# MartinBeseda/FEM-ElastoPlasticity

Measured on NVIDIA B200. Metric: K_tangent assembly Melem/s + DP return-map Mpts/s + PCG-Newton s/step; %HBM roof, higher is better.
Workload: dtype f64

## Files before the change

fem_elastoplasticity_b200/_lib.py:

```python
import ctypes as C
import os

_HERE = os.path.dirname(os.path.abspath(__file__))
LIB_PATH = os.environ.get("FEM_B200_LIB") or os.path.join(_HERE, "libfem_b200.so")

STATUS = {0: "FEM_OK", 1: "FEM_ERR_INVALID_ARG", 2: "FEM_ERR_CUDA", 3: "FEM_ERR_NONFINITE_JACOBIAN",
          4: "FEM_ERR_PCG_BREAKDOWN", 5: "FEM_ERR_PCG_MAXIT", 6: "FEM_ERR_UNSUPPORTED", 7: "FEM_ERR_NO_DEVICE"}
FEM_ERR_PCG_MAXIT = 5


class FemError(RuntimeError):
    def __init__(self, code, msg):
        super().__init__(f"{STATUS.get(code, code)}: {msg}")
        self.code = code


class NonFiniteJacobian(FemError, ArithmeticError):
    pass


_vp, _i64, _i32, _dbl = C.c_void_p, C.c_int64, C.c_int, C.c_double

SIGNATURES = {
    "fem_last_error_string": [],
# ... 27 lines not shown
    "fem_ppcg_begin": [_vp, _vp, _i32, _vp],
    "fem_ppcg_spmv_dot": [_vp, _vp, _vp, _vp, _vp, _vp, C.POINTER(_vp), _i32, _i32, _vp],
    "fem_ppcg_update_xr": [_vp, _vp, _vp, _vp, _vp, _vp, _vp, C.POINTER(_vp), _i32, _i32, _vp],
    "fem_ppcg_update_p": [_vp, _i64, _i64, _vp, _vp, _vp, _i64, _i64, _vp, _i64, _i64, _vp, _vp, C.POINTER(_vp), _i32, _i32, _vp],
    "fem_pcg": [_vp, _vp, _vp, _vp, _dbl, _i32, _i32, _vp, _vp, C.POINTER(_i32), C.POINTER(_dbl), _vp],
    "fem_coarse_galerkin": [_vp, _vp, _vp, _vp, _vp, _dbl, _dbl, _dbl, _dbl, _i32, _i32, _vp, _vp],
    "fem_dense_gemv": [_i32, _vp, _vp, _vp, _vp, _vp],
    "fem_tl_init": [_i64, _vp, _vp, _vp, _vp, _vp, _dbl, _dbl, _dbl, _dbl, _i32, _i32, _vp, _vp, _vp, _vp],
    "fem_tl_update_xr": [_i64, _vp, _vp, _vp, _vp, _dbl, _dbl, _dbl, _dbl, _i32, _i32, _vp, _vp, _vp, _vp, _i32, _vp],
    "fem_tl_apply": [_i64, _i32, _vp, _vp, _vp, _vp, _dbl, _dbl, _dbl, _dbl, _i32, _i32, _vp, _vp, _vp, _i32, _i32, _vp],
    "fem_mg_sizeof": [_i32],
    "fem_mg_lattice": [_i64, _vp, _dbl, _dbl, _dbl, _dbl, _i32, _i32, _i32, _vp, _vp, _vp, _vp],
    "fem_mg_galerkin_fine": [_vp, _vp, _vp, _vp, _vp, _i32, _vp, _i32, _i32, _i32, _i32, _i32, _vp, _vp, _vp],
    "fem_mg_galerkin_stencil": [_i32, _i32, _i32, _i32, _vp, _i32, _i32, _i32, _i32, _i32, _vp, _vp],
    "fem_mg_block_jacobi": [_vp, _vp, _vp, _vp, _vp],
    "fem_mg_level_finalize": [_i64, _vp, _dbl, _vp, _vp],
    "fem_mg_stencil_apply": [_i32, _i32, _i32, _i32, _vp, _vp, _vp, _vp],
    "fem_mg_stencil_to_dense": [_i32, _i32, _vp, _vp, _vp],
    "fem_mg_vcycle": [_vp, _vp, _vp, _vp, _vp, _vp, _vp],
    "fem_peer_allreduce": [_vp, _i32, _vp, C.POINTER(_vp), _i64, _i64, _i64, _i32, _i32, _vp],
    "fem_mg_fine_step": [_vp, _vp, _i32, _vp, _vp, _vp, _vp, _dbl, _dbl, _vp, _vp],
    "fem_mg_to_f32": [_i64, _vp, _vp, _vp],
    "fem_mg_exchange_run": [_vp, _vp, _vp, _vp],
    "fem_mg_pcg_init": [_i64, _vp, _vp, _vp, _vp, _vp, _vp],
    "fem_mg_pcg_update_xr": [_i64, _vp, _vp, _vp, _vp, _vp, _i32, _vp],
    "fem_mg_pcg_update_p": [_i64, _vp, _vp, _vp, _i32, _vp],
    "fem_energy_norms": [_vp, _vp, _vp, _vp, _vp, _vp, _vp, _vp],
    "fem_vec_axpby": [_i64, _dbl, _vp, _dbl, _vp, _vp, _vp],
    "fem_transform": [_vp, _vp, _vp, _vp],
    "fem_vector_volume": [_vp, _vp, C.POINTER(_dbl), _vp, _vp],
    "fem_segment_sum_ordered": [_i64, _vp, _vp, _vp, _vp],
    "fem_midpoints_p2_count": [_i64, _i64, _vp, C.POINTER(_vp), C.POINTER(_i64), C.POINTER(_i64), C.POINTER(_i32), _vp],
    "fem_midpoints_p2_fill": [_vp, _vp, _vp, _vp, _vp, _vp, _vp],
    "fem_midpoints_p2_destroy": [_vp, _vp],
    "fem_set_tuning": [C.c_char_p, _i32],
}
_RESTYPE = {"fem_last_error_string": C.c_char_p, "fem_plan_bytes": _i64}

_lib = None


def load():
    global _lib
    if _lib is not None:
        return _lib
    if not os.path.isfile(LIB_PATH):
        raise ImportError(f"{LIB_PATH} not found: build it with `python -c 'import __graft_entry__ as g; g.build()'` "
                          "(there is no CPU fallback)")
    lib = C.CDLL(LIB_PATH)
    for name, args in SIGNATURES.items():
# ... 6 lines not shown
        if lib.fem_set_tuning(k.strip().encode(), int(v)) != 0:
            raise ValueError(f"FEM_B200_TUNING: unknown key {k!r}")
    return lib


def check(code):
    if code != 0:
        msg = load().fem_last_error_string().decode()
        if code == 3:
            raise NonFiniteJacobian(code, msg)
        raise FemError(code, msg)


def call(name, *args):
    check(getattr(load(), name)(*args))
```

fem_elastoplasticity_b200/csrc/common.cuh:

```cuda
#pragma once
#include <cuda.h>
#include <cuda_runtime.h>
#include <stdint.h>
#include <stdio.h>
#include <string.h>

#include "../../include/fem_b200.h"

#define FEM_MAX_NP 8
#define FEM_MAX_NQ 9
#define FEM_WARP 32
#define FEM_INVALID_KEY 0xFFFFFFFFu
#define FEM_SLICE_COUNTERS 64
#define FEM_SPMV_TILE 256
#define FEM_SPMV_THREADS (2 * FEM_SPMV_TILE)
#define FEM_SPMV_MAXSEG 4
#define FEM_SPMV_CAP 1024
#define FEM_SPMV_DESC 12
#define FEM_STAGE_MAXBOXW 96
int fem_encode_rows_map(CUtensorMap* out, const double* base, int64_t n_int, int rows, int boxw);

void fem_set_error(const char* fmt, ...);

struct FemTuning {
  int return_map_variant;
  int assemble_warps;
  int spmv_group;
  int spmv_blocks_per_sm;
  int assemble_variant;
  int spmv_unroll;
  int spmv_staged;
  int peer_timeout_ms;
  int assemble_canon;
  int strain_variant;
  int mg_stencil_sym;
  int peer_nowait;
};
extern FemTuning g_fem_tuning;

#define FEM_CUDA_CHECK(expr)                                                                     \
  do {                                                                                           \
    cudaError_t _e = (expr);                                                                     \
    if (_e != cudaSuccess) {                                                                     \
      fem_set_error("%s failed at %s:%d: %s", #expr, __FILE__, __LINE__, cudaGetErrorString(_e)); \
      return FEM_ERR_CUDA;                                                                       \
    }                                                                                            \
  } while (0)

#define FEM_REQUIRE(cond, msg)                                    \
  do {                                                            \
// ... 126 lines not shown
```

fem_elastoplasticity_b200/csrc/mg.cu:

```cuda
#include "common.cuh"
#include "spmv.cuh"
#include "spmv_stream.cuh"
#include "peer.cuh"

struct fem_peer_table {
  void* p[FEM_MG_MAX_PEERS];
};

namespace {

struct Geom {
  int nxn, nrows, g0, nrows_global;
  int64_t n;
};
static Geom geom_of(const fem_mg_level& L) { return Geom{L.nxn, L.nrows, L.g0, L.nrows_global, (int64_t)L.nxn * L.nrows}; }

__device__ __forceinline__ double w1(int o) { return o ? 0.5 : 1.0; }

__global__ void mg_lattice_kernel(int64_t n_n, const double* __restrict__ coord, double x0, double y0, double ihx, double ihy, int LX,
                                  int lat_rows, int g0, int32_t* lat, int32_t* __restrict__ node_lat, int32_t* err) {
  for (int64_t a = (int64_t)blockIdx.x * blockDim.x + threadIdx.x; a < n_n; a += (int64_t)gridDim.x * blockDim.x) {
    const double fx = (coord[a] - x0) * ihx, fy = (coord[n_n + a] - y0) * ihy;
    const long long ix = llrint(fx), iy = llrint(fy) - g0;
    if (fabs(fx - (double)ix) > 1e-6 || fabs(fy - (double)(iy + g0)) > 1e-6 || ix < 0 || ix >= LX || iy < 0 || iy >= lat_rows) {
// ... 159 lines not shown
      if (nbr_idx[p0 + j] == a) {
        k00 = vals[4 * (int64_t)p0 + 2 * j];
        k01 = vals[4 * (int64_t)p0 + 2 * j + 1];
        k10 = vals[4 * (int64_t)p0 + 2 * deg + 2 * j];
        k11 = vals[4 * (int64_t)p0 + 2 * deg + 2 * j + 1];
        break;
      }
    const bool f0 = mask ? mask[2 * a] != 0 : true, f1 = mask ? mask[2 * a + 1] != 0 : true;
    double2 ia, ib;
    block_inverse(k00, 0.5 * (k01 + k10), k11, f0, f1, ia, ib);
    dinv[a] = ia;
    dinv[n_n + a] = ib;
  }
}

__global__ void mg_stencil_to_dense_kernel(Geom g, const double* __restrict__ S, double* __restrict__ A) {
  const int64_t t = (int64_t)blockIdx.x * blockDim.x + threadIdx.x;
  if (t >= g.n * 9) return;
  const int64_t node = t / 9;
  const int s = (int)(t % 9);
  const int i = (int)(node % g.nxn), j = (int)(node / g.nxn);
  const int ii = i + s % 3 - 1, jj = j + s / 3 - 1;
  if (ii < 0 || ii >= g.nxn || jj < 0 || jj >= g.nrows) return;
  const int64_t nb = ii + (int64_t)jj * g.nxn, nc = 2 * g.n;
#pragma unroll
  for (int q = 0; q < 4; ++q) A[(2 * node + (q >> 1)) * nc + 2 * nb + (q & 1)] = S[(int64_t)(4 * s + q) * g.n + node];
}

enum { MG_APPLY = 0, MG_RESID = 1, MG_CHEB = 2, MG_FIRST = 3 };

// ... 199 lines not shown
    ordered_accumulate<1>(v, dst, rb);
  }
}

__global__ void __launch_bounds__(256) mg_fine_first_kernel(int64_t lo, int64_t hi, int64_t n_n, const double2* __restrict__ b,
                                                            const double2* __restrict__ dinv, double2* __restrict__ d, double2* __restrict__ out,
                                                            double c2) {
  for (int64_t i = lo + (int64_t)blockIdx.x * blockDim.x + threadIdx.x; i < hi; i += (int64_t)gridDim.x * blockDim.x) {
    const double2 bi = b[i], da = dinv[i], db = dinv[n_n + i];
    const double2 dn = make_double2(c2 * (da.x * bi.x + da.y * bi.y), c2 * (db.x * bi.x + db.y * bi.y));
    d[i] = dn;
    out[i] = dn;
  }
}

template <bool LAT>
__global__ void __launch_bounds__(256) mg_restrict_kernel(Geom c, int row_lo, int row_hi, int nxf, int nrows_f, int g0f, int nrows_global_f,
                                                          const int32_t* __restrict__ lat, const double2* __restrict__ r, double2* __restrict__ bc) {
  const int64_t t = (int64_t)blockIdx.x * blockDim.x + threadIdx.x;
  if (t >= (int64_t)(row_hi - row_lo) * c.nxn) return;
  const int I = (int)(t % c.nxn), J = row_lo + (int)(t / c.nxn), Jg = J + c.g0;
  double a0 = 0.0, a1 = 0.0;
#pragma unroll
  for (int db = -1; db <= 1; ++db) {
    const int fjg = 2 * Jg + db, fj = fjg - g0f;
    if (fjg < 0 || fjg >= nrows_global_f || fj < 0 || fj >= nrows_f) continue;
#pragma unroll
    for (int da = -1; da <= 1; ++da) {
      const int fi = 2 * I + da;
      if (fi < 0 || fi >= nxf) continue;
// ... 37 lines not shown
  const int64_t node = (int64_t)row_lo * f.nxn + t;
  const int i = (int)(node % f.nxn), j = (int)(node / f.nxn);
  const double2 z = prolong_point(c, i, j + f.g0, xc);
  double2 v = xf[node];
  v.x += z.x;
  v.y += z.y;
  xf[node] = v;
}

__global__ void __launch_bounds__(256) mg_prolong_fine_kernel(int64_t n_n, const int32_t* __restrict__ node_lat, int LX, int g0,
                                                              const uint8_t* __restrict__ mask, Geom c, const double2* xc, double2* __restrict__ xf) {
  for (int64_t a = (int64_t)blockIdx.x * blockDim.x + threadIdx.x; a < n_n; a += (int64_t)gridDim.x * blockDim.x) {
    uchar2 mk = make_uchar2(1, 1);
    if (mask) mk = reinterpret_cast<const uchar2*>(mask)[a];
    if (!mk.x && !mk.y) continue;
    const int la = node_lat[a];
    const double2 z = prolong_point(c, la % LX, la / LX + g0, xc);
    double2 v = xf[a];
    if (mk.x) v.x += z.x;
    if (mk.y) v.y += z.y;
    xf[a] = v;
  }
}

__global__ void __launch_bounds__(256) mg_exchange_kernel(const fem_mg_exchange ex, const double2* __restrict__ v, uint64_t* err, uint64_t timeout_ns) {
  __shared__ int sh_last;
  int64_t total = 0;
  for (int k = 0; k < ex.n_send; ++k) total += ex.count[k];
  for (int64_t t = (int64_t)blockIdx.x * blockDim.x + threadIdx.x; t < total; t += (int64_t)gridDim.x * blockDim.x) {
    int64_t o = t;
    int k = 0;
// ... 184 lines not shown
    if (sh.group == 4) MGT(4);
    else if (sh.group == 8) MGT(8);
    else MGT(16);
#undef MGT
  } else {
#define MGR(G) mg_fine_rows_kernel<G, MODE, VT><<<sh.blocks, 256, 0, st>>>(P->n_n, P->nbr_ptr, P->nbr_idx, K, x, epi, dot, rb)
    if (sh.group == 4) MGR(4);
    else if (sh.group == 8) MGR(8);
    else MGR(16);
#undef MGR
  }
  FEM_CUDA_CHECK(cudaGetLastError());
  return FEM_OK;
}

template <int MODE>
int launch_fine(const fem_plan* P, const fem_mg_desc* D, const double* K, const double* b, const double* x, double* out, double c1, double c2,
                double* dot, cudaStream_t st) {
  if (D->K32) return launch_fine_vt<MODE, float>(P, D, D->K32, b, x, out, c1, c2, dot, st);
  return launch_fine_vt<MODE, double>(P, D, K, b, x, out, c1, c2, dot, st);
}

__global__ void __launch_bounds__(256) mg_to_f32_kernel(int64_t n4, const double4* __restrict__ src, float4* __restrict__ dst) {
  for (int64_t i = (int64_t)blockIdx.x * blockDim.x + threadIdx.x; i < n4; i += (int64_t)gridDim.x * blockDim.x) {
    const double2 a = __ldcs(reinterpret_cast<const double2*>(src + i)), b = __ldcs(reinterpret_cast<const double2*>(src + i) + 1);
    __stcs(dst + i, make_float4((float)a.x, (float)a.y, (float)b.x, (float)b.y));
  }
}

#define MG_TRY(expr)             \
  do {                           \
    const int _rc = (expr);      \
    if (_rc != FEM_OK) return _rc; \
// ... 88 lines not shown
  const int64_t items = (int64_t)(row_hi - row_lo) * nxc;
  if (items <= 0) return FEM_OK;
  mg_galerkin_stencil_kernel<<<grid_for(items, 128), 128, 0, (cudaStream_t)stream>>>(f, Sf, c, row_lo, row_hi, Sc);
  FEM_CUDA_CHECK(cudaGetLastError());
  return FEM_OK;
}

extern "C" int fem_mg_block_jacobi(const fem_plan* P, const double* K_vals, const uint8_t* mask, double* dinv, fem_stream stream) {
  FEM_REQUIRE(P && K_vals && dinv, "null pointer");
  mg_block_jacobi_kernel<<<grid_for(P->n_n), 256, 0, (cudaStream_t)stream>>>(P->n_n, P->nbr_ptr, P->nbr_idx, K_vals, mask,
                                                                             reinterpret_cast<double2*>(dinv));
  FEM_CUDA_CHECK(cudaGetLastError());
  return FEM_OK;
}

extern "C" int fem_mg_level_finalize(int64_t n, double* S, double thresh, double* dinv, fem_stream stream) {
  FEM_REQUIRE(S && dinv && n > 0, "null pointer");
  mg_level_finalize_kernel<<<grid_for(n), 256, 0, (cudaStream_t)stream>>>(n, S, thresh, reinterpret_cast<double2*>(dinv));
  FEM_CUDA_CHECK(cudaGetLastError());
  return FEM_OK;
}

extern "C" int fem_mg_stencil_apply(int nxn, int nrows, int row_lo, int row_hi, const double* S, const double* x, double* y, fem_stream stream) {
  FEM_REQUIRE(S && x && y && nxn > 0 && nrows > 0 && row_lo >= 0 && row_hi <= nrows, "null pointer or bad rows");
  const Geom g{nxn, nrows, 0, nrows, (int64_t)nxn * nrows};
  const int64_t items = (int64_t)(row_hi - row_lo) * nxn;
  if (items <= 0) return FEM_OK;
  mg_stencil_kernel<MG_APPLY, double, false><<<grid_for(items), 256, 0, (cudaStream_t)stream>>>(g, row_lo, row_hi, S, reinterpret_cast<const double2*>(x), nullptr,
                                                                                 nullptr, nullptr, reinterpret_cast<double2*>(y), 0.0, 0.0);
  FEM_CUDA_CHECK(cudaGetLastError());
// ... 33 lines not shown
  peer_allreduce_kernel<<<1, 256, 0, (cudaStream_t)stream>>>(vals, n, reinterpret_cast<uint64_t*>(comm), tab, lines_word, seq_word, err_word, rank, world,
                                                            timeout_ns);
  FEM_CUDA_CHECK(cudaGetLastError());
  return FEM_OK;
}

extern "C" int fem_mg_vcycle(const fem_plan* P, const fem_mg_desc* D, const double* K_vals, const double* r, double* z, double* dot,
                             fem_stream stream) {
  FEM_REQUIRE(P && D && K_vals && r && z, "null pointer");
  FEM_REQUIRE(D->n_levels >= 1 && D->n_levels <= FEM_MG_MAX_LEVELS && D->degree >= 1 && D->degree <= FEM_MG_MAX_DEGREE, "levels / degree");
  FEM_REQUIRE(D->lat && D->node_lat && D->dinv && D->xa && D->xb && D->d && D->r && D->coarse_inv, "descriptor");
  FEM_REQUIRE(D->own_node_lo >= 0 && D->own_node_hi <= P->n_n && D->own_node_lo < D->own_node_hi, "owned node range");
  cudaStream_t st = (cudaStream_t)stream;
  const int k = D->degree;
  const int64_t n2 = P->n_n;
  double *cur = D->xa, *oth = D->xb;
  const fem_mg_exchange *ecur = &D->ex_xa, *eoth = &D->ex_xb;
  auto swap = [&]() { double* t = cur; cur = oth; oth = t; const fem_mg_exchange* e = ecur; ecur = eoth; eoth = e; };
  mg_fine_first_kernel<<<vgrid(n2, P->sm_count), 256, 0, st>>>(D->own_node_lo, D->own_node_hi, n2, reinterpret_cast<const double2*>(r), reinterpret_cast<const double2*>(D->dinv),
                                                              reinterpret_cast<double2*>(D->d), reinterpret_cast<double2*>(cur), D->c2[0]);
  FEM_CUDA_CHECK(cudaGetLastError());
  for (int s = 1; s < k; ++s) {
    MG_TRY(run_exchange(*ecur, cur, D->err, st));
    MG_TRY(launch_fine<MG_CHEB>(P, D, K_vals, r, cur, oth, D->c1[s], D->c2[s], nullptr, st));
    swap();
  }
  MG_TRY(run_exchange(*ecur, cur, D->err, st));
  MG_TRY(launch_fine<MG_RESID>(P, D, K_vals, r, cur, D->r, 0.0, 0.0, nullptr, st));
  MG_TRY(run_exchange(D->ex_r, D->r, D->err, st));
  const fem_mg_level& C = D->lev[0];
  {
    const Geom c = geom_of(C);
    const int64_t items = (int64_t)(C.res_hi - C.res_lo) * C.nxn;
    if (items > 0) {
      mg_restrict_kernel<true><<<grid_for(items), 256, 0, st>>>(c, C.res_lo, C.res_hi, D->LX, D->lat_rows, D->g0, D->nrows_global, D->lat,
                                                                reinterpret_cast<const double2*>(D->r), reinterpret_cast<double2*>(C.b));
      FEM_CUDA_CHECK(cudaGetLastError());
    }
    MG_TRY(run_exchange(C.ex_b, C.b, D->err, st));
  }
  const double* xc = nullptr;
  MG_TRY(vcycle_level(D, 0, &xc, st));
  MG_TRY(run_exchange(xc == C.xa ? C.ex_xa : C.ex_xb, xc, D->err, st));
  mg_prolong_fine_kernel<<<vgrid(n2, P->sm_count), 256, 0, st>>>(n2, D->node_lat, D->LX, D->g0, D->mask, geom_of(C), reinterpret_cast<const double2*>(xc),
                                                                reinterpret_cast<double2*>(cur));
  FEM_CUDA_CHECK(cudaGetLastError());
  for (int s = 0; s < k; ++s) {
    const bool last = s == k - 1;
    MG_TRY(run_exchange(*ecur, cur, D->err, st));
    MG_TRY(launch_fine<MG_CHEB>(P, D, K_vals, r, cur, last ? z : oth, s == 0 ? 0.0 : D->c1[s], D->c2[s], last ? dot : nullptr, st));
    swap();
  }
  return FEM_OK;
}

extern "C" int fem_mg_fine_step(const fem_plan* P, const fem_mg_desc* D, int mode, const double* K_vals, const double* b, const double* x,
                                double* out, double c1, double c2, double* dot, fem_stream stream) {
  FEM_REQUIRE(P && D && K_vals && b && x && out && (mode == MG_RESID || mode == MG_CHEB) && out != x, "arguments");
  cudaStream_t st = (cudaStream_t)stream;
// ... 29 lines not shown
```

fem_elastoplasticity_b200/csrc/plan.cu:

```cuda
#include <stdarg.h>

#include <vector>

#include "common.cuh"

static thread_local char g_err[512] = "no error";
void fem_set_error(const char* fmt, ...) {
  va_list ap;
  va_start(ap, fmt);
  vsnprintf(g_err, sizeof(g_err), fmt, ap);
  va_end(ap);
}
extern "C" const char* fem_last_error_string(void) { return g_err; }
extern "C" int fem_version(void) { return 100; }

FemTuning g_fem_tuning = {};
extern "C" int fem_set_tuning(const char* key, int value) {
  FEM_REQUIRE(key != nullptr, "key");
  if (!strcmp(key, "return_map_variant")) g_fem_tuning.return_map_variant = value;
  else if (!strcmp(key, "assemble_warps")) g_fem_tuning.assemble_warps = value;
  else if (!strcmp(key, "spmv_group")) g_fem_tuning.spmv_group = value;
  else if (!strcmp(key, "spmv_blocks_per_sm")) g_fem_tuning.spmv_blocks_per_sm = value;
  else if (!strcmp(key, "assemble_variant")) g_fem_tuning.assemble_variant = value;
  else if (!strcmp(key, "spmv_unroll")) g_fem_tuning.spmv_unroll = value;
  else if (!strcmp(key, "spmv_staged")) g_fem_tuning.spmv_staged = value;
  else if (!strcmp(key, "peer_timeout_ms")) g_fem_tuning.peer_timeout_ms = value;
  else if (!strcmp(key, "peer_nowait")) g_fem_tuning.peer_nowait = value;
  else if (!strcmp(key, "strain_variant")) g_fem_tuning.strain_variant = value;
  else if (!strcmp(key, "assemble_canon")) g_fem_tuning.assemble_canon = value;
  else if (!strcmp(key, "mg_stencil_sym")) g_fem_tuning.mg_stencil_sym = value;
  else {
    fem_set_error("unknown tuning key %s", key);
    return FEM_ERR_INVALID_ARG;
  }
  return FEM_OK;
}

extern "C" int fem_device_info(int* sm_count, int* cc_major, int* cc_minor, int64_t* free_bytes, int64_t* total_bytes) {
  int dev = 0, n = 0;
  if (cudaGetDeviceCount(&n) != cudaSuccess || n == 0) {
    fem_set_error("no CUDA device visible");
    return FEM_ERR_NO_DEVICE;
  }
  FEM_CUDA_CHECK(cudaGetDevice(&dev));
  if (sm_count) FEM_CUDA_CHECK(cudaDeviceGetAttribute(sm_count, cudaDevAttrMultiProcessorCount, dev));
  if (cc_major) FEM_CUDA_CHECK(cudaDeviceGetAttribute(cc_major, cudaDevAttrComputeCapabilityMajor, dev));
  if (cc_minor) FEM_CUDA_CHECK(cudaDeviceGetAttribute(cc_minor, cudaDevAttrComputeCapabilityMinor, dev));
  size_t f = 0, t = 0;
  FEM_CUDA_CHECK(cudaMemGetInfo(&f, &t));
// ... 866 lines not shown
```

fem_elastoplasticity_b200/mg.py:

```python
import ctypes as C
import time

import torch

from ._lib import call, load
from .plan import _ptr, _stream

MAX_LEVELS, MAX_DEGREE, MAX_PEERS = 16, 8, 16


class MultigridUnsupported(ValueError):
    pass


class Exchange(C.Structure):
    _fields_ = [("n_send", C.c_int32), ("n_wait", C.c_int32), ("src_off", C.c_int64 * MAX_PEERS), ("count", C.c_int64 * MAX_PEERS),
                ("dst", C.c_void_p * MAX_PEERS), ("dst_flag", C.c_void_p * MAX_PEERS), ("wait_flag", C.c_void_p * MAX_PEERS),
                ("seq", C.c_void_p)]


class Level(C.Structure):
    _fields_ = [("nxn", C.c_int32), ("nrows", C.c_int32), ("g0", C.c_int32), ("own_lo", C.c_int32), ("own_hi", C.c_int32),
                ("nrows_global", C.c_int32), ("res_lo", C.c_int32), ("res_hi", C.c_int32),
                ("S", C.c_void_p), ("S32", C.c_void_p), ("dinv", C.c_void_p), ("b", C.c_void_p), ("xa", C.c_void_p), ("xb", C.c_void_p), ("d", C.c_void_p),
                ("r", C.c_void_p), ("c1", C.c_double * MAX_DEGREE), ("c2", C.c_double * MAX_DEGREE),
                ("ex_xa", Exchange), ("ex_xb", Exchange), ("ex_r", Exchange), ("ex_b", Exchange)]


class Desc(C.Structure):
    _fields_ = [("n_levels", C.c_int32), ("degree", C.c_int32), ("LX", C.c_int32), ("lat_rows", C.c_int32), ("g0", C.c_int32),
                ("nrows_global", C.c_int32), ("lat", C.c_void_p), ("node_lat", C.c_void_p), ("own_node_lo", C.c_int64),
                ("own_node_hi", C.c_int64), ("mask", C.c_void_p), ("dinv", C.c_void_p), ("xa", C.c_void_p), ("xb", C.c_void_p),
                ("d", C.c_void_p), ("r", C.c_void_p), ("c1", C.c_double * MAX_DEGREE), ("c2", C.c_double * MAX_DEGREE),
                ("ex_xa", Exchange), ("ex_xb", Exchange), ("ex_r", Exchange), ("lev", Level * MAX_LEVELS), ("coarse_inv", C.c_void_p),
                ("K32", C.c_void_p), ("err", C.c_void_p)]


def chebyshev_coefficients(lmax, ratio, degree):
    lmin = lmax / ratio
    theta, delta = 0.5 * (lmax + lmin), 0.5 * (lmax - lmin)
    sigma = theta / delta
    rho = 1.0 / sigma
    c1, c2 = [0.0], [1.0 / theta]
    for _ in range(1, degree):
        rho_new = 1.0 / (2.0 * sigma - rho)
        c1.append(rho_new * rho)
        c2.append(2.0 * rho_new / delta)
        rho = rho_new
    return c1, c2

# ... 102 lines not shown
            self._make_arena(n)
        a = self._vec
        self.r, self.q, self.x, self.z = (z(n) for _ in range(4))
        self.minv = z(2 * n)
        self.p = a("p", n)
        self.scal = z(8)
        self.v0 = {"xa": a("xa0", n), "xb": a("xb0", n), "d": z(n), "r": a("r0", n)}
        self.lv = []
        for li, lay in enumerate(self.layouts):
            g0l, nrows, own_lo, own_hi, res_lo, res_hi = lay["ranks"][rank]
            nn = lay["nxn"] * nrows
            self.lv.append({"nxn": lay["nxn"], "nrows": nrows, "g0": g0l, "own": (own_lo, own_hi), "res": (res_lo, res_hi), "n": nn,
                            "N": lay["nrows_global"], "rep": lay["replicated"], "first_rep": lay["first_replicated"],
                            "S": z(36 * nn), "dinv": z(4 * nn), "d": z(2 * nn), "b": a(f"b{li + 1}", 2 * nn),
                            "xa": a(f"xa{li + 1}", 2 * nn), "xb": a(f"xb{li + 1}", 2 * nn), "r": a(f"r{li + 1}", 2 * nn), "lmax": None})
        self.coarse_inv, self.desc, self.setup_seconds, self.lmax0 = None, None, None, None
        self._graph, self._graph_key = None, None
        self.launches_last = 0

    def _vec(self, name, size):
        if name in self._arena_slots:
            off, _ = self._arena_slots[name]
            return self.arena[off:off + size]
        return torch.zeros(size, dtype=torch.float64, device=self.device)

    def _make_arena(self, n):
        import torch.distributed as dist
        import torch.distributed._symmetric_memory as symm
        dev, world = self.device, self.world
        nmax = torch.tensor([n], dtype=torch.int64, device=dev)
# ... 132 lines not shown
        for li in range(1, self.n_levels):
            f, c = self.lv[li - 1], self.lv[li]
            rows = c["res"] if c["first_rep"] else c["own"]
            call("fem_mg_galerkin_stencil", f["nxn"], f["nrows"], f["g0"], f["N"], _ptr(f["S"]), c["nxn"], c["nrows"], c["g0"], rows[0], rows[1],
                 _ptr(c["S"]), _stream())
            if self.part is not None:
                if c["first_rep"]:
                    dist.all_reduce(c["S"])
                elif not c["rep"]:
                    self._halo_rows(c, c["S"].view(36, c["nrows"], c["nxn"]))
        for lv in self.lv:
            nn = lv["n"]
            dmax = torch.maximum(lv["S"][16 * nn:17 * nn].max(), lv["S"][19 * nn:20 * nn].max()).reshape(1)
            self._all_reduce(dmax, op=None if self.part is None else dist.ReduceOp.MAX)
            call("fem_mg_level_finalize", nn, _ptr(lv["S"]), 1e-14 * float(dmax.item()), _ptr(lv["dinv"]), _stream())
        self.lmax0 = 1.1 * self._power_fine(k_vals)
        for lv in self.lv[:-1]:
            lv["lmax"] = 1.1 * self._power_level(lv)
        last = self.lv[-1]
        nc = 2 * last["n"]
        A = torch.empty((nc, nc), dtype=torch.float64, device=dev)
        call("fem_mg_stencil_to_dense", last["nxn"], last["nrows"], _ptr(last["S"]), _ptr(A), _stream())
        A = 0.5 * (A + A.t())
        self.coarse_inv = torch.cholesky_inverse(torch.linalg.cholesky(A)).contiguous()
        v = torch.randn((nc, 4), dtype=torch.float64, device=dev, generator=torch.Generator(device=dev).manual_seed(7))
        self.inverse_residual = float(((A @ (self.coarse_inv @ v)) - v).norm() / v.norm())
        if not self.inverse_residual <= 1e-6:
            raise ArithmeticError(f"multigrid: dense inverse of the coarsest operator is inaccurate (residual {self.inverse_residual:.2e})")
        del A
        self._build_desc()
        torch.cuda.synchronize()
        self.setup_seconds = time.perf_counter() - t0
        return self

    @staticmethod
    def block_apply(dinv, v):
        n = v.numel()
        a, b, v2 = dinv[:n].view(-1, 2), dinv[n:2 * n].view(-1, 2), v.view(-1, 2)
        return torch.stack([a[:, 0] * v2[:, 0] + a[:, 1] * v2[:, 1], b[:, 0] * v2[:, 0] + b[:, 1] * v2[:, 1]], dim=1).reshape(-1)

    def block_jacobi(self, k_vals, out=None):
        out = self.minv if out is None else out
        call("fem_mg_block_jacobi", self.plan._h, _ptr(k_vals), _ptr(self.mask), _ptr(out), _stream())
        return out

    def _power_fine(self, k_vals, iters=20):
        P = self.plan
        dinv = self.block_jacobi(k_vals)
        g = torch.Generator(device=self.device).manual_seed(11 + self.rank)
        v = torch.randn(P.n_dof, dtype=torch.float64, device=self.device, generator=g) * self.mask
        y = torch.empty_like(v)
        lam = 1.0
        for _ in range(iters):
            if self.part is not None:
                self.part.halo_exchange(v)
            P.spmv(k_vals, v, mask=self.mask, out=y)
# ... 39 lines not shown
            L = d.lev[li]
            L.nxn, L.nrows, L.g0, L.own_lo, L.own_hi, L.nrows_global = lv["nxn"], lv["nrows"], lv["g0"], lv["own"][0], lv["own"][1], lv["N"]
            L.res_lo, L.res_hi = lv["res"]
            L.S, L.dinv = lv["S"].data_ptr(), lv["dinv"].data_ptr()
            if self.k32 is not None and li < self.n_levels - 1:
                lv["S32"] = lv["S"].to(torch.float32)
                L.S32 = lv["S32"].data_ptr()
            L.b, L.xa, L.xb, L.d, L.r = (lv[k].data_ptr() for k in ("b", "xa", "xb", "d", "r"))
            if lv["lmax"] is not None:
                c1, c2 = chebyshev_coefficients(lv["lmax"], self.ratio, self.degree)
                for k in range(self.degree):
                    L.c1[k], L.c2[k] = c1[k], c2[k]
        d.coarse_inv = self.coarse_inv.data_ptr()
        d.K32 = self.k32.data_ptr() if self.k32 is not None else 0
        d.err = 0
        self._fill_exchanges(d)
        self.desc = d

    def _fill_exchanges(self, d):
        if self.part is None:
            return
        p, LX = self.part, self.lattice[4]
        rows0 = [(r * p.ny_loc, p.ny_loc + 1 + (1 if r < self.world - 1 else 0), 1 if r > 0 else 0, p.ny_loc + 1) for r in range(self.world)]
        d.ex_xa, d.ex_xb, d.ex_r = (self._halo_desc(k, LX, rows0) for k in ("xa0", "xb0", "r0"))
        self.ex_p = self._halo_desc("p", LX, rows0)
        for li, lay in enumerate(self.layouts):
            L = d.lev[li]
            if not lay["replicated"]:
                rr = [rk[:4] for rk in lay["ranks"]]
                L.ex_xa, L.ex_xb, L.ex_r = (self._halo_desc(f"{k}{li + 1}", lay["nxn"], rr) for k in ("xa", "xb", "r"))
# ... 37 lines not shown
        self._sum_scal(3, 4)
        call("fem_mg_pcg_update_xr", n, _ptr(self.p), _ptr(self.q), _ptr(self.x), _ptr(self.r), _ptr(s), it, _stream())
        slot = 0 if it & 1 else 2
        self.vcycle(k_vals, self.r, self.z, s[slot:slot + 1])
        self._sum_scal(*((1, 3) if it % 2 == 0 else (0, 2)))
        self._update_p(it)

    def launches_per_iteration(self):
        k, L = self.degree, self.n_levels
        return 3 + (2 * k + 3) + (L - 1) * (2 * k + 3) + 1

    def solve(self, k_vals, rhs, rtol=1e-10, maxit=500, check_every=2, iters=None):
        if self.desc is None:
            self.setup(k_vals)
        P, s, n = self.plan, self.scal, self.plan.n_dof
        self.block_jacobi(k_vals)
        if self.k32 is not None:
            call("fem_mg_to_f32", P.nnz, _ptr(k_vals), _ptr(self.k32), _stream())
        call("fem_mg_pcg_init", n, _ptr(rhs), _ptr(self.mask), _ptr(self.r), _ptr(self.x), _ptr(s), _stream())
        self._sum_scal(0, 5)
        self.vcycle(k_vals, self.r, self.z, s[0:1])
        self._sum_scal(0, 1)
        self._update_p(-1)
        n_it = iters if iters is not None else maxit
        it, rel = 0, float("inf")
        h = s.cpu()
        bb = float(h[4])
        if iters is None and (bb == 0.0 or float(h[1]) <= rtol * rtol * bb):
            return self.x, 0, 0.0 if bb == 0.0 else (float(h[1]) / bb) ** 0.5
        graph = None
        if self.use_graph and n_it >= 4:
            if self._graph is None or self._graph_key != k_vals.data_ptr():
                self._iteration(k_vals, 0)
                self._iteration(k_vals, 1)
                it = 2
                self._capture_pair(k_vals)
            graph = self._graph
        self.launches_last = 0
        hint = getattr(self, "_hint_iters", {}).get(rtol)
        skip_until = 0 if iters is not None else check_schedule(hint, check_every)
        while it < n_it:
            nxt = n_it if iters is not None else next_check(it, n_it, check_every, skip_until)
            while it < nxt:
                if graph is not None and it % 2 == 0 and it + 2 <= nxt:
                    graph.replay()
                    it += 2
                else:
                    self._iteration(k_vals, it)
                    it += 1
            h = s.cpu()
            self.check_peer_error()
            if not torch.isfinite(h[1]):
                raise ArithmeticError("multigrid PCG breakdown: residual is not finite")
            rel = float((h[1] / h[4]).sqrt()) if h[4] > 0 else 0.0
            if iters is None and rel <= rtol:
                break
        self.launches_last = it * self.launches_per_iteration()
        if self.part is not None:
            self.part.halo_exchange(self.x)
        if iters is None and not rel <= rtol:
            from .distributed import PCGNotConverged
            raise PCGNotConverged("multigrid PCG", it, rel, rtol)
        if iters is None:
            self.__dict__.setdefault("_hint_iters", {})[rtol] = it
        return self.x, it, rel

    def _capture_pair(self, k_vals):
        try:
            torch.cuda.synchronize()
            g = torch.cuda.CUDAGraph()
            with torch.cuda.graph(g):
                self._iteration(k_vals, 0)
                self._iteration(k_vals, 1)
            self._graph, self._graph_key = g, k_vals.data_ptr()
        except Exception as e:
            self.graph_error, self.use_graph, self._graph = repr(e), False, None
```

include/fem_b200.h:

```cpp
#ifndef FEM_B200_H
#define FEM_B200_H

#include <stdint.h>

#ifdef __cplusplus
extern "C" {
#endif

typedef struct fem_plan fem_plan;
typedef void* fem_stream;

typedef enum fem_status {
  FEM_OK = 0,
  FEM_ERR_INVALID_ARG = 1,
  FEM_ERR_CUDA = 2,
  FEM_ERR_NONFINITE_JACOBIAN = 3,
  FEM_ERR_PCG_BREAKDOWN = 4,
  FEM_ERR_PCG_MAXIT = 5,
  FEM_ERR_UNSUPPORTED = 6,
  FEM_ERR_NO_DEVICE = 7
} fem_status;

const char* fem_last_error_string(void);
int fem_version(void);
// ... 96 lines not shown
typedef struct fem_mg_desc {
  int32_t n_levels, degree;
  int32_t LX, lat_rows, g0, nrows_global;
  const int32_t* lat;
  const int32_t* node_lat;
  int64_t own_node_lo, own_node_hi;
  const uint8_t* mask;
  const double* dinv;
  double *xa, *xb, *d, *r;
  double c1[FEM_MG_MAX_DEGREE], c2[FEM_MG_MAX_DEGREE];
  fem_mg_exchange ex_xa, ex_xb, ex_r;
  fem_mg_level lev[FEM_MG_MAX_LEVELS];
  const double* coarse_inv;
  const float* K32;
  uint64_t* err;
} fem_mg_desc;
int fem_mg_sizeof(int which);
int fem_mg_lattice(int64_t n_n, const double* coord, double x0, double y0, double hx, double hy, int LX, int lat_rows, int g0,
                   int32_t* lat, int32_t* node_lat, int32_t* err, fem_stream stream);
int fem_mg_galerkin_fine(const fem_plan* plan, const double* K_vals, const uint8_t* row_mask, const uint8_t* col_mask,
                         const int32_t* lat, int lat_rows, const int32_t* node_lat, int LX, int g0, int nxn, int nrows, int g0c,
                         double* S, int32_t* err, fem_stream stream);
int fem_mg_galerkin_stencil(int nxf, int nrows_f, int g0f, int nrows_global_f, const double* Sf, int nxc, int nrows_c, int g0c,
                            int row_lo, int row_hi, double* Sc, fem_stream stream);
int fem_mg_level_finalize(int64_t n, double* S, double thresh, double* dinv, fem_stream stream);
int fem_mg_block_jacobi(const fem_plan* plan, const double* K_vals, const uint8_t* mask, double* dinv, fem_stream stream);
int fem_mg_stencil_apply(int nxn, int nrows, int row_lo, int row_hi, const double* S, const double* x, double* y, fem_stream stream);
int fem_mg_stencil_to_dense(int nxn, int nrows, const double* S, double* A, fem_stream stream);
int fem_mg_vcycle(const fem_plan* plan, const fem_mg_desc* desc, const double* K_vals, const double* r, double* z, double* dot,
                  fem_stream stream);
#define FEM_PEER_ALLREDUCE_WORDS 512
int fem_peer_allreduce(double* vals, int n, void* comm, const void* const* peers, int64_t lines_word, int64_t seq_word, int64_t err_word,
                       int rank, int world, fem_stream stream);
int fem_mg_fine_step(const fem_plan* plan, const fem_mg_desc* desc, int mode, const double* K_vals, const double* b, const double* x,
                     double* out, double c1, double c2, double* dot, fem_stream stream);
int fem_mg_to_f32(int64_t n, const double* src, float* dst, fem_stream stream);
int fem_mg_exchange_run(const fem_mg_exchange* ex, double* v, uint64_t* err, fem_stream stream);
int fem_mg_pcg_init(int64_t n, const double* rhs, const uint8_t* mask, double* r, double* x, double* scal, fem_stream stream);
int fem_mg_pcg_update_xr(int64_t n, const double* p, const double* q, double* x, double* r, double* scal, int iter, fem_stream stream);
int fem_mg_pcg_update_p(int64_t n, const double* z, double* p, double* scal, int iter, fem_stream stream);

// ... 1 lines not shown
                     double* work, double* out, fem_stream stream);

int fem_vec_axpby(int64_t n, double a, const double* x, double b, const double* y, double* out, fem_stream stream);
int fem_transform(const fem_plan* plan, const double* q_int, double* q_node, fem_stream stream);

int fem_vector_volume(const fem_plan* plan, const double* f_int, const double* h_hatp, double* out, fem_stream stream);
int fem_segment_sum_ordered(int64_t n_seg, const int64_t* seg_ptr, const double* vals, double* out, fem_stream stream);

int fem_midpoints_p2_count(int64_t n_n, int64_t n_e, const int32_t* elem, void** handle, int64_t* n_mid, int64_t* n_bnd,
                           int* status, fem_stream stream);
int fem_midpoints_p2_fill(void* handle, const double* coord, double* coord_mid, int32_t* elem_mid, int32_t* edge_el,
                          int32_t* surf, fem_stream stream);
int fem_midpoints_p2_destroy(void* handle, fem_stream stream);

int fem_set_tuning(const char* key, int value);

#ifdef __cplusplus
}
#endif
#endif
```

Measured before the change: 20400.

## Apply fine-level multigrid smoother as structured lattice stencil in float32 planes

Result: no change. 20470, median of 6 (+0.4%).

```diff
diff --git a/fem_elastoplasticity_b200/_lib.py b/fem_elastoplasticity_b200/_lib.py
--- a/fem_elastoplasticity_b200/_lib.py
+++ b/fem_elastoplasticity_b200/_lib.py
@@ -65,6 +65,7 @@
     "fem_mg_galerkin_fine": [_vp, _vp, _vp, _vp, _vp, _i32, _vp, _i32, _i32, _i32, _i32, _i32, _vp, _vp, _vp],
     "fem_mg_galerkin_stencil": [_i32, _i32, _i32, _i32, _vp, _i32, _i32, _i32, _i32, _i32, _vp, _vp],
     "fem_mg_block_jacobi": [_vp, _vp, _vp, _vp, _vp],
+    "fem_mg_lattice_prepare": [_vp, _vp, _vp, _vp, _i32, _i32, _vp, _vp, _vp, _vp],
     "fem_mg_level_finalize": [_i64, _vp, _dbl, _vp, _vp],
     "fem_mg_stencil_apply": [_i32, _i32, _i32, _i32, _vp, _vp, _vp, _vp],
     "fem_mg_stencil_to_dense": [_i32, _i32, _vp, _vp, _vp],
@@ -85,6 +86,7 @@
     "fem_midpoints_p2_fill": [_vp, _vp, _vp, _vp, _vp, _vp, _vp],
     "fem_midpoints_p2_destroy": [_vp, _vp],
     "fem_set_tuning": [C.c_char_p, _i32],
+    "fem_get_tuning": [C.c_char_p, C.POINTER(_i32)],
 }
 _RESTYPE = {"fem_last_error_string": C.c_char_p, "fem_plan_bytes": _i64}
 
@@ -121,3 +123,9 @@
 
 def call(name, *args):
     check(getattr(load(), name)(*args))
+
+
+def get_tuning(key):
+    v = _i32(0)
+    call("fem_get_tuning", key.encode(), C.byref(v))
+    return v.value
diff --git a/fem_elastoplasticity_b200/csrc/common.cuh b/fem_elastoplasticity_b200/csrc/common.cuh
--- a/fem_elastoplasticity_b200/csrc/common.cuh
+++ b/fem_elastoplasticity_b200/csrc/common.cuh
@@ -34,6 +34,7 @@
   int assemble_canon;
   int strain_variant;
   int mg_stencil_sym;
+  int mg_fine_lattice;
   int peer_nowait;
 };
 extern FemTuning g_fem_tuning;
diff --git a/fem_elastoplasticity_b200/csrc/mg.cu b/fem_elastoplasticity_b200/csrc/mg.cu
--- a/fem_elastoplasticity_b200/csrc/mg.cu
+++ b/fem_elastoplasticity_b200/csrc/mg.cu
@@ -2,6 +2,8 @@
 #include "spmv.cuh"
 #include "spmv_stream.cuh"
 #include "peer.cuh"
+
+#include <algorithm>
 
 struct fem_peer_table {
   void* p[FEM_MG_MAX_PEERS];
@@ -197,6 +199,67 @@
   }
 }
 
+constexpr int MG_LAT_PLANES = 15;
+__global__ void __launch_bounds__(256) mg_lattice_prepare_kernel(int64_t n_n, const int32_t* __restrict__ nbr_ptr, const int32_t* __restrict__ nbr_idx,
+                                                                 const double* __restrict__ vals, const uint8_t* __restrict__ mask,
+                                                                 const int32_t* __restrict__ node_lat, int LX, int diag, float* __restrict__ S,
+                                                                 double2* __restrict__ dinv, int32_t* err) {
+  for (int64_t a = (int64_t)blockIdx.x * blockDim.x + threadIdx.x; a < n_n; a += (int64_t)gridDim.x * blockDim.x) {
+    int bad = (node_lat && node_lat[a] != a) ? 1 : 0;
+    const int p0 = nbr_ptr[a], deg = nbr_ptr[a + 1] - p0;
+    const double* row0 = vals + 4 * (int64_t)p0;
+    const double* row1 = row0 + 2 * deg;
+    const double m0 = mask ? (double)(mask[2 * a] != 0) : 1.0, m1 = mask ? (double)(mask[2 * a + 1] != 0) : 1.0;
+    const int ia = (int)(a % LX), ja = (int)(a / LX);
+    double k00 = 0.0, k01 = 0.0, k10 = 0.0, k11 = 0.0;
+    float s[MG_LAT_PLANES];
+#pragma unroll
+    for (int q = 0; q < MG_LAT_PLANES; ++q) s[q] = 0.0f;
+    for (int j = 0; j < deg; ++j) {
+      const int b = nbr_idx[p0 + j];
+      const int dx = b % LX - ia, dy = b / LX - ja;
+      const double v00 = row0[2 * j], v01 = row0[2 * j + 1], v10 = row1[2 * j], v11 = row1[2 * j + 1];
+      if (b == a) {
+        k00 = v00;
+        k01 = v01;
+        k10 = v10;
+        k11 = v11;
+        s[0] = (float)(v00 * m0);
+        s[1] = (float)(v01 * (m0 * m1));
+        s[2] = (float)(v11 * m1);
+        continue;
+      }
+      int dir = -1;
+      if (dy == 0 && dx == 1) dir = 0;
+      else if (dy == 1 && dx == 0) dir = 1;
+      else if (dy == 1 && (dx == 1 || dx == -1)) {
+        if (diag == 0) bad |= dx == 1 ? 4 : 8;
+        else if (dx == diag) dir = 2;
+        else bad |= 2;
+      } else if (!((dy == 0 && dx == -1) || (dy == -1 && dx == 0) || (dy == -1 && (diag == 0 ? (dx == 1 || dx == -1) : dx == -diag)))) {
+        bad |= 2;
+      }
+      if (dir < 0) continue;
+      const double n0 = mask ? (double)(mask[2 * (int64_t)b] != 0) : 1.0, n1 = mask ? (double)(mask[2 * (int64_t)b + 1] != 0) : 1.0;
+      s[3 + 4 * dir] = (float)(v00 * (m0 * n0));
+      s[4 + 4 * dir] = (float)(v01 * (m0 * n1));
+      s[5 + 4 * dir] = (float)(v10 * (m1 * n0));
+      s[6 + 4 * dir] = (float)(v11 * (m1 * n1));
+    }
+    if (bad && err) atomicOr(err, bad);
+    if (S) {
+#pragma unroll
+      for (int q = 0; q < MG_LAT_PLANES; ++q) S[(int64_t)q * n_n + a] = s[q];
+    }
+    if (dinv) {
+      double2 ia2, ib2;
+      block_inverse(k00, 0.5 * (k01 + k10), k11, m0 != 0.0, m1 != 0.0, ia2, ib2);
+      dinv[a] = ia2;
+      dinv[n_n + a] = ib2;
+    }
+  }
+}
+
 __global__ void mg_stencil_to_dense_kernel(Geom g, const double* __restrict__ S, double* __restrict__ A) {
   const int64_t t = (int64_t)blockIdx.x * blockDim.x + threadIdx.x;
   if (t >= g.n * 9) return;
@@ -426,6 +489,73 @@
   }
 }
 
+template <int MODE, int MINB>
+__global__ void __launch_bounds__(256, MINB) mg_lattice_sweep_kernel(int64_t n, int LX, int NY, int diag, const float* __restrict__ S, const double2* x,
+                                                               const double2* __restrict__ b, const double2* __restrict__ dinv, double2* d,
+                                                               double2* out, const uint8_t* __restrict__ mask, double c1, double c2,
+                                                               double* dot_out, const FemRedBuf rb) {
+  __shared__ double red[32];
+  double dot = 0.0;
+  for (int64_t a = (int64_t)blockIdx.x * blockDim.x + threadIdx.x; a < n; a += (int64_t)gridDim.x * blockDim.x) {
+    const int i = (int)a % LX, j = (int)a / LX;
+    const float* sp = S + a;
+    const double2 xa = x[a];
+    const double s01 = (double)__ldg(sp + n);
+    double y0 = fma((double)__ldg(sp), xa.x, s01 * xa.y);
+    double y1 = fma((double)__ldg(sp + 2 * n), xa.y, s01 * xa.x);
+#pragma unroll
+    for (int k = 0; k < 3; ++k) {
+      const int dx = k == 0 ? 1 : (k == 1 ? 0 : diag), dy = k == 0 ? 0 : 1;
+      const int64_t off = (int64_t)dy * LX + dx;
+      const bool vf = i + dx >= 0 && i + dx < LX && j + dy < NY, vb = i - dx >= 0 && i - dx < LX && j - dy >= 0;
+      {
+        const float* q = sp + (int64_t)(3 + 4 * k) * n;
+        const double2 xv = vf ? x[a + off] : make_double2(0.0, 0.0);
+        y0 = fma((double)__ldg(q), xv.x, y0);
+        y0 = fma((double)__ldg(q + n), xv.y, y0);
+        y1 = fma((double)__ldg(q + 2 * n), xv.x, y1);
+        y1 = fma((double)__ldg(q + 3 * n), xv.y, y1);
+      }
+      {
+        const int64_t c = vb ? a - off : a;
+        const float* q = S + (int64_t)(3 + 4 * k) * n + c;
+        const double2 xv = vb ? x[c] : make_double2(0.0, 0.0);
+        y0 = fma((double)__ldg(q), xv.x, y0);
+        y0 = fma((double)__ldg(q + 2 * n), xv.y, y0);
+        y1 = fma((double)__ldg(q + n), xv.x, y1);
+        y1 = fma((double)__ldg(q + 3 * n), xv.y, y1);
+      }
+    }
+    const double2 bi = b[a];
+    double r0 = bi.x - y0, r1 = bi.y - y1;
+    if (MODE == MG_RESID) {
+      if (mask) {
+        const uchar2 mk = reinterpret_cast<const uchar2*>(mask)[a];
+        if (!mk.x) r0 = 0.0;
+        if (!mk.y) r1 = 0.0;
+      }
+      out[a] = make_double2(r0, r1);
+      continue;
+    }
+    const double2 da = dinv[a], db = dinv[n + a];
+    double2 dn = make_double2(c2 * (da.x * r0 + da.y * r1), c2 * (db.x * r0 + db.y * r1));
+    if (c1 != 0.0) {
+      const double2 dd = d[a];
+      dn.x = fma(c1, dd.x, dn.x);
+      dn.y = fma(c1, dd.y, dn.y);
+    }
+    d[a] = dn;
+    const double2 xo = make_double2(xa.x + dn.x, xa.y + dn.y);
+    out[a] = xo;
+    if (MODE == MG_CHEB && dot_out) dot = fma(bi.x, xo.x, fma(bi.y, xo.y, dot));
+  }
+  if (MODE == MG_CHEB && dot_out) {
+    const double v[1] = {block_sum(dot, red)};
+    double* const dst[1] = {dot_out};
+    ordered_accumulate<1>(v, dst, rb);
+  }
+}
+
 template <bool LAT>
 __global__ void __launch_bounds__(256) mg_restrict_kernel(Geom c, int row_lo, int row_hi, int nxf, int nrows_f, int g0f, int nrows_global_f,
                                                           const int32_t* __restrict__ lat, const double2* __restrict__ r, double2* __restrict__ bc) {
@@ -493,7 +623,7 @@
     uchar2 mk = make_uchar2(1, 1);
     if (mask) mk = reinterpret_cast<const uchar2*>(mask)[a];
     if (!mk.x && !mk.y) continue;
-    const int la = node_lat[a];
+    const int la = node_lat ? node_lat[a] : (int)a;
     const double2 z = prolong_point(c, la % LX, la / LX + g0, xc);
     double2 v = xf[a];
     if (mk.x) v.x += z.x;
@@ -708,9 +838,29 @@
   return FEM_OK;
 }
 
+bool fine_on_lattice(const fem_mg_desc* D) { return D->S0 != nullptr && g_fem_tuning.mg_fine_lattice != 2; }
+
+template <int MODE>
+int launch_lattice(const fem_plan* P, const fem_mg_desc* D, const double* b, const double* x, double* out, double c1, double c2, double* dot,
+                   cudaStream_t st) {
+  const int64_t n = P->n_n;
+  FEM_REQUIRE(D->LX > 0 && (int64_t)D->LX * D->lat_rows == n && D->g0 == 0 && D->own_node_lo == 0 && D->own_node_hi == n &&
+                  (D->S0_diag == 1 || D->S0_diag == -1),
+              "lattice stencil descriptor (one GPU, node id = lattice point)");
+  const unsigned blocks = (unsigned)std::min<int64_t>((n + 255) / 256, FEM_RED_MAXB);
+  const FemRedBuf rb{P->red_partials, P->red_ticket};
+  constexpr int minb = MODE == MG_RESID ? 6 : 4;
+  mg_lattice_sweep_kernel<MODE, minb><<<blocks, 256, 0, st>>>(n, D->LX, D->lat_rows, D->S0_diag, D->S0, reinterpret_cast<const double2*>(x),
+                                                              reinterpret_cast<const double2*>(b), reinterpret_cast<const double2*>(D->dinv),
+                                                              reinterpret_cast<double2*>(D->d), reinterpret_cast<double2*>(out), D->mask, c1, c2, dot, rb);
+  FEM_CUDA_CHECK(cudaGetLastError());
+  return FEM_OK;
+}
+
 template <int MODE>
 int launch_fine(const fem_plan* P, const fem_mg_desc* D, const double* K, const double* b, const double* x, double* out, double c1, double c2,
                 double* dot, cudaStream_t st) {
+  if (fine_on_lattice(D)) return launch_lattice<MODE>(P, D, b, x, out, c1, c2, dot, st);
   if (D->K32) return launch_fine_vt<MODE, float>(P, D, D->K32, b, x, out, c1, c2, dot, st);
   return launch_fine_vt<MODE, double>(P, D, K, b, x, out, c1, c2, dot, st);
 }
@@ -829,6 +979,15 @@
   return FEM_OK;
 }
 
+extern "C" int fem_mg_lattice_prepare(const fem_plan* P, const double* K_vals, const uint8_t* mask, const int32_t* node_lat, int LX, int diag,
+                                      float* S0, double* dinv, int32_t* err, fem_stream stream) {
+  FEM_REQUIRE(P && K_vals && LX > 0 && P->n_n % LX == 0 && diag >= -1 && diag <= 1 && (S0 == nullptr || diag != 0), "lattice prepare arguments");
+  mg_lattice_prepare_kernel<<<grid_for(P->n_n), 256, 0, (cudaStream_t)stream>>>(P->n_n, P->nbr_ptr, P->nbr_idx, K_vals, mask, node_lat, LX, diag, S0,
+                                                                                reinterpret_cast<double2*>(dinv), err);
+  FEM_CUDA_CHECK(cudaGetLastError());
+  return FEM_OK;
+}
+
 extern "C" int fem_mg_level_finalize(int64_t n, double* S, double thresh, double* dinv, fem_stream stream) {
   FEM_REQUIRE(S && dinv && n > 0, "null pointer");
   mg_level_finalize_kernel<<<grid_for(n), 256, 0, (cudaStream_t)stream>>>(n, S, thresh, reinterpret_cast<double2*>(dinv));
@@ -892,6 +1051,7 @@
   cudaStream_t st = (cudaStream_t)stream;
   const int k = D->degree;
   const int64_t n2 = P->n_n;
+  const bool lat_ids = fine_on_lattice(D);
   double *cur = D->xa, *oth = D->xb;
   const fem_mg_exchange *ecur = &D->ex_xa, *eoth = &D->ex_xb;
   auto swap = [&]() { double* t = cur; cur = oth; oth = t; const fem_mg_exchange* e = ecur; ecur = eoth; eoth = e; };
@@ -911,8 +1071,12 @@
     const Geom c = geom_of(C);
     const int64_t items = (int64_t)(C.res_hi - C.res_lo) * C.nxn;
     if (items > 0) {
-      mg_restrict_kernel<true><<<grid_for(items), 256, 0, st>>>(c, C.res_lo, C.res_hi, D->LX, D->lat_rows, D->g0, D->nrows_global, D->lat,
-                                                                reinterpret_cast<const double2*>(D->r), reinterpret_cast<double2*>(C.b));
+      if (lat_ids)
+        mg_restrict_kernel<false><<<grid_for(items), 256, 0, st>>>(c, C.res_lo, C.res_hi, D->LX, D->lat_rows, D->g0, D->nrows_global, nullptr,
+                                                                   reinterpret_cast<const double2*>(D->r), reinterpret_cast<double2*>(C.b));
+      else
+        mg_restrict_kernel<true><<<grid_for(items), 256, 0, st>>>(c, C.res_lo, C.res_hi, D->LX, D->lat_rows, D->g0, D->nrows_global, D->lat,
+                                                                  reinterpret_cast<const double2*>(D->r), reinterpret_cast<double2*>(C.b));
       FEM_CUDA_CHECK(cudaGetLastError());
     }
     MG_TRY(run_exchange(C.ex_b, C.b, D->err, st));
@@ -920,7 +1084,7 @@
   const double* xc = nullptr;
   MG_TRY(vcycle_level(D, 0, &xc, st));
   MG_TRY(run_exchange(xc == C.xa ? C.ex_xa : C.ex_xb, xc, D->err, st));
-  mg_prolong_fine_kernel<<<vgrid(n2, P->sm_count), 256, 0, st>>>(n2, D->node_lat, D->LX, D->g0, D->mask, geom_of(C), reinterpret_cast<const double2*>(xc),
+  mg_prolong_fine_kernel<<<vgrid(n2, P->sm_count), 256, 0, st>>>(n2, lat_ids ? nullptr : D->node_lat, D->LX, D->g0, D->mask, geom_of(C), reinterpret_cast<const double2*>(xc),
                                                                 reinterpret_cast<double2*>(cur));
   FEM_CUDA_CHECK(cudaGetLastError());
   for (int s = 0; s < k; ++s) {
diff --git a/fem_elastoplasticity_b200/csrc/plan.cu b/fem_elastoplasticity_b200/csrc/plan.cu
--- a/fem_elastoplasticity_b200/csrc/plan.cu
+++ b/fem_elastoplasticity_b200/csrc/plan.cu
@@ -15,24 +15,41 @@
 extern "C" int fem_version(void) { return 100; }
 
 FemTuning g_fem_tuning = {};
+static int* tuning_slot(const char* key) {
+  struct Entry {
+    const char* key;
+    int* slot;
+  };
+  static const Entry table[] = {{"return_map_variant", &g_fem_tuning.return_map_variant}, {"assemble_warps", &g_fem_tuning.assemble_warps},
+                                {"spmv_group", &g_fem_tuning.spmv_group},                 {"spmv_blocks_per_sm", &g_fem_tuning.spmv_blocks_per_sm},
+                                {"assemble_variant", &g_fem_tuning.assemble_variant},     {"spmv_unroll", &g_fem_tuning.spmv_unroll},
+                                {"spmv_staged", &g_fem_tuning.spmv_staged},               {"peer_timeout_ms", &g_fem_tuning.peer_timeout_ms},
+                                {"peer_nowait", &g_fem_tuning.peer_nowait},               {"strain_variant", &g_fem_tuning.strain_variant},
+                                {"assemble_canon", &g_fem_tuning.assemble_canon},         {"mg_stencil_sym", &g_fem_tuning.mg_stencil_sym},
+                                {"mg_fine_lattice", &g_fem_tuning.mg_fine_lattice}};
+  if (key == nullptr) return nullptr;
+  for (const Entry& e : table)
+    if (!strcmp(key, e.key)) return e.slot;
+  return nullptr;
+}
 extern "C" int fem_set_tuning(const char* key, int value) {
   FEM_REQUIRE(key != nullptr, "key");
-  if (!strcmp(key, "return_map_variant")) g_fem_tuning.return_map_variant = value;
-  else if (!strcmp(key, "assemble_warps")) g_fem_tuning.assemble_warps = value;
-  else if (!strcmp(key, "spmv_group")) g_fem_tuning.spmv_group = value;
-  else if (!strcmp(key, "spmv_blocks_per_sm")) g_fem_tuning.spmv_blocks_per_sm = value;
-  else if (!strcmp(key, "assemble_variant")) g_fem_tuning.assemble_variant = value;
-  else if (!strcmp(key, "spmv_unroll")) g_fem_tuning.spmv_unroll = value;
-  else if (!strcmp(key, "spmv_staged")) g_fem_tuning.spmv_staged = value;
-  else if (!strcmp(key, "peer_timeout_ms")) g_fem_tuning.peer_timeout_ms = value;
-  else if (!strcmp(key, "peer_nowait")) g_fem_tuning.peer_nowait = value;
-  else if (!strcmp(key, "strain_variant")) g_fem_tuning.strain_variant = value;
-  else if (!strcmp(key, "assemble_canon")) g_fem_tuning.assemble_canon = value;
-  else if (!strcmp(key, "mg_stencil_sym")) g_fem_tuning.mg_stencil_sym = value;
-  else {
+  int* slot = tuning_slot(key);
+  if (!slot) {
     fem_set_error("unknown tuning key %s", key);
     return FEM_ERR_INVALID_ARG;
   }
+  *slot = value;
+  return FEM_OK;
+}
+extern "C" int fem_get_tuning(const char* key, int* value) {
+  FEM_REQUIRE(key != nullptr && value != nullptr, "key / value");
+  const int* slot = tuning_slot(key);
+  if (!slot) {
+    fem_set_error("unknown tuning key %s", key);
+    return FEM_ERR_INVALID_ARG;
+  }
+  *value = *slot;
   return FEM_OK;
 }
 
diff --git a/fem_elastoplasticity_b200/mg.py b/fem_elastoplasticity_b200/mg.py
--- a/fem_elastoplasticity_b200/mg.py
+++ b/fem_elastoplasticity_b200/mg.py
@@ -3,7 +3,7 @@
 
 import torch
 
-from ._lib import call, load
+from ._lib import call, get_tuning, load
 from .plan import _ptr, _stream
 
 MAX_LEVELS, MAX_DEGREE, MAX_PEERS = 16, 8, 16
@@ -33,7 +33,7 @@
                 ("own_node_hi", C.c_int64), ("mask", C.c_void_p), ("dinv", C.c_void_p), ("xa", C.c_void_p), ("xb", C.c_void_p),
                 ("d", C.c_void_p), ("r", C.c_void_p), ("c1", C.c_double * MAX_DEGREE), ("c2", C.c_double * MAX_DEGREE),
                 ("ex_xa", Exchange), ("ex_xb", Exchange), ("ex_r", Exchange), ("lev", Level * MAX_LEVELS), ("coarse_inv", C.c_void_p),
-                ("K32", C.c_void_p), ("err", C.c_void_p)]
+                ("K32", C.c_void_p), ("err", C.c_void_p), ("S0", C.c_void_p), ("S0_diag", C.c_int32), ("S0_pad", C.c_int32)]
 
 
 def chebyshev_coefficients(lmax, ratio, degree):
@@ -166,6 +166,7 @@
                             "N": lay["nrows_global"], "rep": lay["replicated"], "first_rep": lay["first_replicated"],
                             "S": z(36 * nn), "dinv": z(4 * nn), "d": z(2 * nn), "b": a(f"b{li + 1}", 2 * nn),
                             "xa": a(f"xa{li + 1}", 2 * nn), "xb": a(f"xb{li + 1}", 2 * nn), "r": a(f"r{li + 1}", 2 * nn), "lmax": None})
+        self.s0, self.s0_diag = None, 0
         self.coarse_inv, self.desc, self.setup_seconds, self.lmax0 = None, None, None, None
         self._graph, self._graph_key = None, None
         self.launches_last = 0
@@ -328,6 +329,7 @@
             dmax = torch.maximum(lv["S"][16 * nn:17 * nn].max(), lv["S"][19 * nn:20 * nn].max()).reshape(1)
             self._all_reduce(dmax, op=None if self.part is None else dist.ReduceOp.MAX)
             call("fem_mg_level_finalize", nn, _ptr(lv["S"]), 1e-14 * float(dmax.item()), _ptr(lv["dinv"]), _stream())
+        self._setup_fine_lattice(k_vals)
         self.lmax0 = 1.1 * self._power_fine(k_vals)
         for lv in self.lv[:-1]:
             lv["lmax"] = 1.1 * self._power_level(lv)
@@ -353,7 +355,29 @@
         a, b, v2 = dinv[:n].view(-1, 2), dinv[n:2 * n].view(-1, 2), v.view(-1, 2)
         return torch.stack([a[:, 0] * v2[:, 0] + a[:, 1] * v2[:, 1], b[:, 0] * v2[:, 0] + b[:, 1] * v2[:, 1]], dim=1).reshape(-1)
 
+    def _setup_fine_lattice(self, k_vals):
+        self.s0, self.s0_diag = None, 0
+        P, LX, NY = self.plan, self.lattice[4], self.lattice[5]
+        if self.k32 is None or self.part is not None or P.n_n != LX * NY:
+            return
+        if not bool((self.node_lat == torch.arange(P.n_n, dtype=torch.int32, device=self.device)).all()):
+            return
+        err = torch.zeros(1, dtype=torch.int32, device=self.device)
+        call("fem_mg_lattice_prepare", P._h, _ptr(k_vals), _ptr(self.mask), _ptr(self.node_lat), LX, 0, None, None, _ptr(err), _stream())
+        e = int(err.item())
+        if e & 3 or (e & 12) == 12:
+            return
+        self.s0_diag = -1 if e & 8 else 1
+        self.s0 = torch.zeros(15 * P.n_n, dtype=torch.float32, device=self.device)
+
+    def fine_lattice_active(self):
+        return self.s0 is not None and get_tuning("mg_fine_lattice") != 2
+
     def block_jacobi(self, k_vals, out=None):
+        if out is None and self.fine_lattice_active():
+            call("fem_mg_lattice_prepare", self.plan._h, _ptr(k_vals), _ptr(self.mask), None, self.lattice[4], self.s0_diag, _ptr(self.s0),
+                 _ptr(self.minv), None, _stream())
+            return self.minv
         out = self.minv if out is None else out
         call("fem_mg_block_jacobi", self.plan._h, _ptr(k_vals), _ptr(self.mask), _ptr(out), _stream())
         return out
@@ -423,6 +447,7 @@
         d.coarse_inv = self.coarse_inv.data_ptr()
         d.K32 = self.k32.data_ptr() if self.k32 is not None else 0
         d.err = 0
+        d.S0, d.S0_diag = (self.s0.data_ptr(), self.s0_diag) if self.s0 is not None else (0, 0)
         self._fill_exchanges(d)
         self.desc = d
 
@@ -490,8 +515,9 @@
         if self.desc is None:
             self.setup(k_vals)
         P, s, n = self.plan, self.scal, self.plan.n_dof
+        lattice = self.fine_lattice_active()
         self.block_jacobi(k_vals)
-        if self.k32 is not None:
+        if self.k32 is not None and not lattice:
             call("fem_mg_to_f32", P.nnz, _ptr(k_vals), _ptr(self.k32), _stream())
         call("fem_mg_pcg_init", n, _ptr(rhs), _ptr(self.mask), _ptr(self.r), _ptr(self.x), _ptr(s), _stream())
         self._sum_scal(0, 5)
@@ -506,11 +532,11 @@
             return self.x, 0, 0.0 if bb == 0.0 else (float(h[1]) / bb) ** 0.5
         graph = None
         if self.use_graph and n_it >= 4:
-            if self._graph is None or self._graph_key != k_vals.data_ptr():
+            if self._graph is None or self._graph_key != (k_vals.data_ptr(), lattice):
                 self._iteration(k_vals, 0)
                 self._iteration(k_vals, 1)
                 it = 2
-                self._capture_pair(k_vals)
+                self._capture_pair(k_vals, lattice)
             graph = self._graph
         self.launches_last = 0
         hint = getattr(self, "_hint_iters", {}).get(rtol)
@@ -541,13 +567,13 @@
             self.__dict__.setdefault("_hint_iters", {})[rtol] = it
         return self.x, it, rel
 
-    def _capture_pair(self, k_vals):
+    def _capture_pair(self, k_vals, lattice):
         try:
             torch.cuda.synchronize()
             g = torch.cuda.CUDAGraph()
             with torch.cuda.graph(g):
                 self._iteration(k_vals, 0)
                 self._iteration(k_vals, 1)
-            self._graph, self._graph_key = g, k_vals.data_ptr()
+            self._graph, self._graph_key = g, (k_vals.data_ptr(), lattice)
         except Exception as e:
             self.graph_error, self.use_graph, self._graph = repr(e), False, None
diff --git a/include/fem_b200.h b/include/fem_b200.h
--- a/include/fem_b200.h
+++ b/include/fem_b200.h
@@ -134,6 +134,9 @@
   const double* coarse_inv;
   const float* K32;
   uint64_t* err;
+  const float* S0;
+  int32_t S0_diag;
+  int32_t S0_pad;
 } fem_mg_desc;
 int fem_mg_sizeof(int which);
 int fem_mg_lattice(int64_t n_n, const double* coord, double x0, double y0, double hx, double hy, int LX, int lat_rows, int g0,
@@ -145,6 +148,8 @@
                             int row_lo, int row_hi, double* Sc, fem_stream stream);
 int fem_mg_level_finalize(int64_t n, double* S, double thresh, double* dinv, fem_stream stream);
 int fem_mg_block_jacobi(const fem_plan* plan, const double* K_vals, const uint8_t* mask, double* dinv, fem_stream stream);
+int fem_mg_lattice_prepare(const fem_plan* plan, const double* K_vals, const uint8_t* mask, const int32_t* node_lat, int LX, int diag,
+                           float* S0, double* dinv, int32_t* err, fem_stream stream);
 int fem_mg_stencil_apply(int nxn, int nrows, int row_lo, int row_hi, const double* S, const double* x, double* y, fem_stream stream);
 int fem_mg_stencil_to_dense(int nxn, int nrows, const double* S, double* A, fem_stream stream);
 int fem_mg_vcycle(const fem_plan* plan, const fem_mg_desc* desc, const double* K_vals, const double* r, double* z, double* dot,
@@ -176,6 +181,7 @@
 int fem_midpoints_p2_destroy(void* handle, fem_stream stream);
 
 int fem_set_tuning(const char* key, int value);
+int fem_get_tuning(const char* key, int* value);
 
 #ifdef __cplusplus
 }
```
